# rferguson22/Gaussian-Process

Hardware: AMD Instinct MI355X
Metric: PSO objective evals/sec (swarm x iters) at N=4096 d=3 (higher is better)
Workload: dtype f64; 1 GPU; PSO objective, BASELINE config C: synthetic N=4096 d=3, swarm 64/GPU x 1 GPU = 64; N=4096, d=3, swarm=64, swarm_per_gpu=64, global_batch=64, seq_len=4096, parallelism=single GPU, hetero_noise=False, particles=interior l~U[0.05,0.6]^d (full work)

## Files before the change

gaussian-process_amd/csrc/gpf_common.hip:

```cpp
#pragma once

#include <hip/hip_runtime.h>
#include <stdint.h>

#include <utility>

namespace gpf {

typedef double d4 __attribute__((ext_vector_type(4)));
typedef double d2 __attribute__((ext_vector_type(2)));

constexpr int NTHR = 256;
constexpr int DNTH = 512;
constexpr int T = 128;
constexpr int DMAX = 32;
constexpr int KGRID_MAX = 4096;

__device__ __forceinline__ d4 mfma(double a, double b, d4 c) {
  return __builtin_amdgcn_mfma_f64_16x16x4f64(a, b, c, 0, 0, 0);
}

template <int TM> struct TileCfg;
template <> struct TileCfg<128> {
  static constexpr int KC = 16, NW = 8, WR = 1, WC = 8;
};

template <int TM> struct Geo {
  static constexpr int KC = TileCfg<TM>::KC;
  static constexpr int NW = TileCfg<TM>::NW;
  static constexpr int WR = TileCfg<TM>::WR;
  static constexpr int WC = TileCfg<TM>::WC;
  static constexpr int NTH = 64 * NW;
  static constexpr int MBR = TM / WR / 16;
  static constexpr int MBC = TM / WC / 16;
  static_assert(WR * WC == NW, "wave grid");
};

template <int TM> struct Quad {
  int lane, rb, cb;
  __device__ Quad() {
    const int tid = threadIdx.x;
    lane = tid & 63;
    const int w = __builtin_amdgcn_readfirstlane(tid >> 6);
    if constexpr (Geo<TM>::WR == 1) {
      rb = 0;
      cb = (w >= 4 ? 11 - w : w) * (TM / Geo<TM>::WC);
    } else {
      const int wr = w / Geo<TM>::WC, wc = w % Geo<TM>::WC;
      rb = wr * (TM / Geo<TM>::WR);
      cb = ((wr & 1) ? (Geo<TM>::WC - 1 - wc) : wc) * (TM / Geo<TM>::WC);
    }
  }
  __device__ __forceinline__ int row(int mi, int r) const { return rb + mi * 16 + (lane >> 4) + 4 * r; }
  __device__ __forceinline__ int col(int ni) const { return cb + ni * 16 + (lane & 15); }
};

template <typename P>
__device__ __forceinline__ P* launder(P* p) {
  using G = __attribute__((address_space(1))) P*;
  G g = (G)p;
  asm volatile("" : "+v"(g));
  return (P*)g;
}

template <int TM> struct Acc {
  static constexpr int MBR = Geo<TM>::MBR, MBC = Geo<TM>::MBC;
  d4 v[MBR][MBC];
  __device__ __forceinline__ void zero() {
#pragma unroll
    for (int i = 0; i < MBR; ++i)
#pragma unroll
      for (int j = 0; j < MBC; ++j) v[i][j] = d4{0.0, 0.0, 0.0, 0.0};
  }
  template <typename F>
  __device__ __forceinline__ void foreach(const Quad<TM>& q, F f) const {
#pragma unroll
    for (int mi = 0; mi < MBR; ++mi)
#pragma unroll
      for (int ni = 0; ni < MBC; ++ni)
#pragma unroll
        for (int r = 0; r < 4; ++r) f(q.row(mi, r), q.col(ni), v[mi][ni][r]);
  }
  __device__ __forceinline__ void load(const Quad<TM>& q, const double* base, size_t ld) {
    const double* p0 = launder(base + (size_t)(q.rb + (q.lane >> 4)) * ld + q.cb + (q.lane & 15));
#pragma unroll
    for (int mi = 0; mi < MBR; ++mi)
#pragma unroll
      for (int ni = 0; ni < MBC; ++ni)
#pragma unroll
        for (int r = 0; r < 4; ++r) v[mi][ni][r] = p0[(size_t)(mi * 16 + 4 * r) * ld + ni * 16];
  }
  __device__ __forceinline__ void store(const Quad<TM>& q, double* base, size_t ld) const {
    double* p0 = launder(base + (size_t)(q.rb + (q.lane >> 4)) * ld + q.cb + (q.lane & 15));
#pragma unroll
    for (int mi = 0; mi < MBR; ++mi)
#pragma unroll
      for (int ni = 0; ni < MBC; ++ni)
#pragma unroll
        for (int r = 0; r < 4; ++r) p0[(size_t)(mi * 16 + 4 * r) * ld + ni * 16] = v[mi][ni][r];
  }
  __device__ __forceinline__ void store_wt(const Quad<TM>& q, double* base, size_t ld) const {
    using G = __attribute__((address_space(1))) unsigned long long*;
    G p0 = (G)launder(base + (size_t)(q.rb + (q.lane >> 4)) * ld + q.cb + (q.lane & 15));
#pragma unroll
    for (int mi = 0; mi < MBR; ++mi)
#pragma unroll
      for (int ni = 0; ni < MBC; ++ni)
#pragma unroll
        for (int r = 0; r < 4; ++r)
          __hip_atomic_store(p0 + (size_t)(mi * 16 + 4 * r) * ld + ni * 16,
                             (unsigned long long)__double_as_longlong(v[mi][ni][r]), __ATOMIC_RELAXED,
                             __HIP_MEMORY_SCOPE_AGENT);
  }
  template <typename F>
  __device__ __forceinline__ void visit(const Quad<TM>& q, double* base, size_t ld, F f) const {
    double* p0 = launder(base + (size_t)(q.rb + (q.lane >> 4)) * ld + q.cb + (q.lane & 15));
#pragma unroll
    for (int mi = 0; mi < MBR; ++mi)
#pragma unroll
      for (int ni = 0; ni < MBC; ++ni)
#pragma unroll
        for (int r = 0; r < 4; ++r) f(p0[(size_t)(mi * 16 + 4 * r) * ld + ni * 16], v[mi][ni][r]);
  }
};

enum Tri : int {
  TRI_NONE = 0,
  TRI_B_KLEC,
  TRI_B_KGEC,
  TRI_A_KLER,
  TRI_C_LOWER,
  TRI_A_LAST,
};

template <int TRI>
__device__ __forceinline__ bool tri_live(int R0, int C0, int k) {
  if (TRI == TRI_B_KLEC) return k <= C0 + 15;
  if (TRI == TRI_B_KGEC) return k + 3 >= C0;
  if (TRI == TRI_A_KLER) return k <= R0 + 15;
  if (TRI == TRI_C_LOWER) return C0 <= R0 + 15;
  return true;
}

constexpr int DL_KC = 16;
constexpr int DL_BUF = 2 * 128 * DL_KC;
constexpr int DL_STAGE = 2 * DL_BUF;

__device__ __forceinline__ d4 mfma_neg_a(double a, double b, d4 c) {
  return __builtin_amdgcn_mfma_f64_16x16x4f64(a, b, c, 0, 0, 1);
}

__device__ __forceinline__ void dl_load(const double* g, double* l) {
  const uint32_t m = (uint32_t)(uintptr_t)(__attribute__((address_space(3))) void*)l;
  asm volatile("s_nop 0\n\tglobal_load_lds_dwordx4 %0, off" ::"v"(g), "{m0}"(m) : "memory");
}
template <bool NT = false>
__device__ __forceinline__ void dl_load_s(const void* base, uint32_t off, double* l) {
  const uint32_t m = (uint32_t)(uintptr_t)(__attribute__((address_space(3))) void*)l;
  if constexpr (NT)
    asm volatile("s_nop 0\n\tglobal_load_lds_dwordx4 %0, %1 nt" ::"v"(off), "s"(base), "{m0}"(m) : "memory");
  else
    asm volatile("s_nop 0\n\tglobal_load_lds_dwordx4 %0, %1" ::"v"(off), "s"(base), "{m0}"(m) : "memory");
}
#ifndef GPF_SUM_SHFL
#define GPF_SUM_SHFL 0
#endif
#ifndef GPF_B_NT
#define GPF_B_NT 1
#endif

__device__ __forceinline__ int dl_sw(int r) { return (r >> 1) & 7; }

template <typename P>
__device__ __forceinline__ P* uniform_ptr(P* p) {
  const unsigned long long v = (unsigned long long)(uintptr_t)p;
  const unsigned lo = __builtin_amdgcn_readfirstlane((unsigned)v), hi = __builtin_amdgcn_readfirstlane((unsigned)(v >> 32));
  return (P*)(uintptr_t)(((unsigned long long)hi << 32) | lo);
}

__device__ __forceinline__ void dl_row_offsets(int lane, uint32_t (&o)[4]) {
  const int lr = lane & 15, lk = lane >> 4;
#pragma unroll
  for (int s = 0; s < 4; ++s) o[s] = 8u * (uint32_t)(lr * DL_KC + 2 * ((2 * s + (lk >> 1)) ^ dl_sw(lr)) + (lk & 1));
}

template <bool NN, bool NEG, int NS = 2, bool BNT = true, bool TN = false>
struct DenseRun {
  static_assert(NS >= 2 && NS <= 4, "DenseRun stages");
  static_assert(!TN || NN, "TN: both operands are [k][c] panels");
  static constexpr int MBR = Geo<128>::MBR;
  static_assert(Geo<128>::MBC == 1 && Geo<128>::WR == 1, "128-tile wave layout: all rows x one column slab");
  uint32_t la[4], lb[4];
  uint32_t ga[2], gb[2];
  int blk0;

  __device__ __forceinline__ DenseRun(const Quad<128>& qd, int lda, int ldb, int wave) {
    const int lane = qd.lane, lr = lane & 15, lk = lane >> 4;
    if constexpr (TN) {
#pragma unroll
      for (int mi = 0; mi < 4; ++mi) la[mi] = 8u * (uint32_t)(lk * 128 + 2 * (8 * (mi ^ lk) + (lr >> 1)) + (lr & 1));
    } else {
      dl_row_offsets(lane, la);
    }
    if (!NN) {
#pragma unroll
      for (int s = 0; s < 4; ++s) lb[s] = la[s] + 8u * (uint32_t)(128 * DL_KC + qd.cb * DL_KC);
    } else {
      const int col = qd.cb + lr;
      lb[0] = 8u * (uint32_t)(128 * DL_KC + lk * 128 + 2 * ((col >> 1) ^ (8 * (lk & 3))) + (col & 1));
      lb[1] = lb[2] = lb[3] = lb[0];
    }
    blk0 = 2 * wave;
#pragma unroll
    for (int u = 0; u < 2; ++u) {
      const int blk = blk0 + u, row = 8 * blk + (lane >> 3), kp = (lane & 7) ^ dl_sw(row);
      ga[u] = TN ? 8u * (uint32_t)(blk * ldb + 2 * (lane ^ (8 * (blk & 3)))) : 8u * (uint32_t)(row * lda + 2 * kp);
      gb[u] = NN ? 8u * (uint32_t)(blk * ldb + 2 * (lane ^ (8 * (blk & 3)))) : 8u * (uint32_t)(row * ldb + 2 * kp);
    }
  }

  template <int BUF>
  __device__ __forceinline__ void issue(const double* Ap, const double* Bp, int ldb, int c, double* smem) const {
    const char* Ac = uniform_ptr(TN ? (const char*)(Ap + (size_t)c * DL_KC * ldb) : (const char*)(Ap + c * DL_KC));
    const char* Bc = uniform_ptr(NN ? (const char*)(Bp + (size_t)c * DL_KC * ldb) : (const char*)(Bp + c * DL_KC));
    double* sbuf = smem + BUF * DL_BUF;
#pragma unroll
    for (int u = 0; u < 2; ++u) {
      const int blk = blk0 + u;
      dl_load_s(Ac, ga[u], sbuf + (TN ? blk * 128 : blk * 8 * DL_KC));
      dl_load_s<BNT && GPF_B_NT != 0>(Bc, gb[u], sbuf + 128 * DL_KC + (NN ? blk * 128 : blk * 8 * DL_KC));
    }
  }

  template <int M0>
  __device__ __forceinline__ void reads(const char* sb, int s, double (&a)[MBR], double& b) const {
#pragma unroll
    for (int mi = M0; mi < MBR; ++mi) {
      if constexpr (TN) a[mi] = *(const double*)(sb + la[mi & 3] + (mi >> 2) * 64 * 8 + s * 512 * 8);
      else a[mi] = *(const double*)(sb + la[s] + mi * 16 * DL_KC * 8);
    }
    b = NN ? *(const double*)(sb + lb[0] + s * 512 * 8) : *(const double*)(sb + lb[s]);
  }

  template <int BUF, int M0>
  __device__ __forceinline__ void mma(Acc<128>& acc, const double* smem) const {
    if constexpr (M0 >= MBR) return;
    const char* sb = (const char*)smem + BUF * DL_BUF * 8;
    double a[MBR], b;
    reads<M0>(sb, 0, a, b);
#pragma unroll
    for (int s = 0; s < 4; ++s) {
#pragma unroll
      for (int mi = M0; mi < MBR; ++mi) acc.v[mi][0] = NEG ? mfma_neg_a(a[mi], b, acc.v[mi][0]) : mfma(a[mi], b, acc.v[mi][0]);
      if (s < 3) reads<M0>(sb, s + 1, a, b);
    }
  }

  template <int BUF, int M0>
  __device__ __forceinline__ void chunk(Acc<128>& acc, const double* Ap, const double* Bp, int ldb, int t, int nch,
                                        double* smem) const {
    if constexpr (NS == 2) {
      asm volatile("s_waitcnt vmcnt(0)" ::: "memory");
    } else {
      if (t + NS - 2 < nch) {
        if constexpr (NS == 3) asm volatile("s_waitcnt vmcnt(4)" ::: "memory");
        else asm volatile("s_waitcnt vmcnt(8)" ::: "memory");
      } else {
        asm volatile("s_waitcnt vmcnt(0)" ::: "memory");
      }
    }
    __syncthreads();
    if (t + NS - 1 < nch) issue<(BUF + NS - 1) % NS>(Ap, Bp, ldb, t + NS - 1, smem);
    mma<BUF, M0>(acc, smem);
  }
  template <int M0>
  __device__ __forceinline__ void chunk_rt(int b, Acc<128>& acc, const double* Ap, const double* Bp, int ldb, int t,
                                           int nch, double* smem) const {
    switch (b) {
      case 0: chunk<0, M0>(acc, Ap, Bp, ldb, t, nch, smem); break;
      case 1: chunk<1 % NS, M0>(acc, Ap, Bp, ldb, t, nch, smem); break;
      case 2: chunk<2 % NS, M0>(acc, Ap, Bp, ldb, t, nch, smem); break;
      default: chunk<3 % NS, M0>(acc, Ap, Bp, ldb, t, nch, smem); break;
    }
  }

  template <int M0>
  __device__ __forceinline__ void run(Acc<128>& acc, const double* Ap, const double* Bp, int ldb, int t0, int t1,
                                      int nch, double* smem) const {
    int t = t0;
    if constexpr (NS == 2) {
      if (t < t1 && (t & 1)) chunk<1, M0>(acc, Ap, Bp, ldb, t++, nch, smem);
#pragma unroll 1
      for (; t + 1 < t1; t += 2) {
        chunk<0, M0>(acc, Ap, Bp, ldb, t, nch, smem);
        chunk<1, M0>(acc, Ap, Bp, ldb, t + 1, nch, smem);
      }
      if (t < t1) chunk<0, M0>(acc, Ap, Bp, ldb, t, nch, smem);
    } else {
#pragma unroll 1
      for (; t < t1 && t % NS != 0; ++t) chunk_rt<M0>(t % NS, acc, Ap, Bp, ldb, t, nch, smem);
#pragma unroll 1
      for (; t + NS - 1 < t1; t += NS) {
        chunk<0, M0>(acc, Ap, Bp, ldb, t, nch, smem);
        chunk<1, M0>(acc, Ap, Bp, ldb, t + 1, nch, smem);
        chunk<2 % NS, M0>(acc, Ap, Bp, ldb, t + 2, nch, smem);
        if constexpr (NS == 4) chunk<3, M0>(acc, Ap, Bp, ldb, t + 3, nch, smem);
      }
#pragma unroll 1
      for (; t < t1; ++t) chunk_rt<M0>(t % NS, acc, Ap, Bp, ldb, t, nch, smem);
    }
  }
};

template <bool NN, bool NEG = false, int TRI = TRI_NONE, int NS = 2, bool BNT = true, bool TN = false>
__device__ __forceinline__ void gemm_stream_dl(Acc<128>& acc, const double* __restrict__ Ap, int lda, const double* __restrict__ Bp,
                               int ldb, int K, double* smem, const Quad<128>& qd) {
  const int nch = K / DL_KC;
  if (nch <= 0) return;
  const int wave = __builtin_amdgcn_readfirstlane(threadIdx.x >> 6);
  const double* Ar = uniform_ptr(Ap);
  const double* Br = uniform_ptr(Bp);
  const DenseRun<NN, NEG, NS, BNT, TN> dr(qd, lda, ldb, wave);
  dr.template issue<0>(Ar, Br, ldb, 0, smem);
  if constexpr (NS >= 3) {
    if (nch > 1) dr.template issue<1>(Ar, Br, ldb, 1, smem);
    if constexpr (NS >= 4)
      if (nch > 2) dr.template issue<2>(Ar, Br, ldb, 2, smem);
  }
  __builtin_amdgcn_s_waitcnt(0x0F70);
#define GPF_RUN(m0, a, b) dr.template run<m0>(acc, Ar, Br, ldb, (a), (b), nch, smem)
  const int slab = qd.cb / 16;
  if constexpr (TRI == TRI_NONE) {
    GPF_RUN(0, 0, nch);
// ... 78 lines not shown
#pragma unroll
  for (int mi = M0; mi < 8; ++mi)
#pragma unroll
    for (int r = 0; r < 4; ++r) {
      double* q = p1 + (size_t)(mi * 16 + 4 * r) * ldc;
      if (WT)
        __hip_atomic_store(reinterpret_cast<unsigned long long*>(q),
                           (unsigned long long)__double_as_longlong(acc.v[mi][0][r]), __ATOMIC_RELAXED,
                           __HIP_MEMORY_SCOPE_AGENT);
      else
        *q = acc.v[mi][0][r];
    }
}

template <bool WT>
__device__ __forceinline__ void syrk_tile(double* __restrict__ C, size_t ldc, const double* __restrict__ A, int lda,
                                          int K, double* smem, const Quad<128>& qd) {
  switch (qd.cb / 16) {
    case 0: syrk_rows<WT, 0>(C, ldc, A, lda, K, smem, qd); break;
    case 1: syrk_rows<WT, 1>(C, ldc, A, lda, K, smem, qd); break;
    case 2: syrk_rows<WT, 2>(C, ldc, A, lda, K, smem, qd); break;
    case 3: syrk_rows<WT, 3>(C, ldc, A, lda, K, smem, qd); break;
    case 4: syrk_rows<WT, 4>(C, ldc, A, lda, K, smem, qd); break;
    case 5: syrk_rows<WT, 5>(C, ldc, A, lda, K, smem, qd); break;
    case 6: syrk_rows<WT, 6>(C, ldc, A, lda, K, smem, qd); break;
    default: syrk_rows<WT, 7>(C, ldc, A, lda, K, smem, qd); break;
  }
}

constexpr int TRI_LD = 17;
constexpr int TRI_LDS = 36 * 16 * TRI_LD;
__host__ __device__ constexpr int tri_chunk(int m) { return 16 * TRI_LD * (8 * m - m * (m - 1) / 2); }

__device__ __forceinline__ int tri_row_chunk(int ri, int& rr) {
  int m = 0, base = 0;
#pragma unroll
  for (int mm = 0; mm < 7; ++mm)
    if (ri >= base + 16 * (8 - m)) {
      base += 16 * (8 - m);
      ++m;
    }
  rr = ri - base;
  return m;
}
struct NoHook {
  __device__ void operator()() const {}
};
#ifndef GPF_TRI_STAGE_SCALAR
#define GPF_TRI_STAGE_SCALAR 1
#endif
__host__ __device__ __forceinline__ void tri_block(int b, int& m, int& rb) {
  m = 0;
  int base = 0;
#pragma unroll
  for (int mm = 0; mm < 7; ++mm)
    if (b >= base + (8 - m)) {
      base += 8 - m;
      ++m;
    }
  rb = m + (b - base);
}
template <typename Hook = NoHook>
__device__ __forceinline__ void tri_to_lds(const double* __restrict__ U, size_t ld, double* s, Hook hook = Hook()) {
#if GPF_TRI_STAGE_SCALAR
  {
    const int tid = threadIdx.x;
    const int grp = __builtin_amdgcn_readfirstlane(tid >> 7);
    const int r = (tid >> 3) & 15, kp = tid & 7;
    const double* ul = U + (size_t)r * ld + 2 * kp;
    d2 v[9];
#pragma unroll
    for (int u = 0; u < 9; ++u) {
      int m, rb;
      tri_block(grp + 4 * u, m, rb);
      v[u] = *reinterpret_cast<const d2*>(ul + (size_t)(16 * rb) * ld + 16 * m);
    }
    if constexpr (!__is_same(Hook, NoHook)) {
      asm volatile("s_waitcnt vmcnt(0)" ::: "memory");
      hook();
    }
    double* sl = s + r * TRI_LD + 2 * kp;
#pragma unroll
    for (int u = 0; u < 9; ++u) {
      int m, rb;
      tri_block(grp + 4 * u, m, rb);
      const int off = tri_chunk(m) + 16 * (rb - m) * TRI_LD;
      sl[off] = v[u].x;
      sl[off + 1] = v[u].y;
    }
    __syncthreads();
    return;
  }
#endif
  int tid = threadIdx.x;
  d2 v[9];
#pragma unroll
  for (int u = 0; u < 9; ++u) {
    const int i = tid + DNTH * u, ri = i >> 3, kp = i & 7;
    int rr;
    const int m = tri_row_chunk(ri, rr);
    v[u] = *reinterpret_cast<const d2*>(U + (size_t)(16 * m + rr) * ld + 16 * m + 2 * kp);
  }
  if constexpr (!__is_same(Hook, NoHook)) {
    asm volatile("s_waitcnt vmcnt(0)" ::: "memory");
    hook();
  }
  asm volatile("" : "+v"(tid));
#pragma unroll
  for (int u = 0; u < 9; ++u) {
    const int i = tid + DNTH * u, ri = i >> 3, kp = i & 7;
    int rr;
    const int m = tri_row_chunk(ri, rr);
    const int dst = tri_chunk(m) + rr * TRI_LD + 2 * kp;
    s[dst] = v[u].x;
    s[dst + 1] = v[u].y;
  }
  __syncthreads();
}

template <int P, bool NEG>
__device__ __forceinline__ void trmm_acc(d4 (&out)[2], const Acc<128>& X, const double* sU) {
  constexpr int NQ = 4 * (2 * P + 2);
  const int lane = threadIdx.x & 63;
  const uint32_t b0 = 8u * (uint32_t)((lane & 15) * TRI_LD + (lane >> 4));
  uint32_t b1 = b0 + 32768u;
  asm volatile("" : "+v"(b1));
  const char* u = (const char*)sU;
  out[0] = d4{0.0, 0.0, 0.0, 0.0};
  out[1] = d4{0.0, 0.0, 0.0, 0.0};
  double a[2][2];
  auto reads = [&](int q, double (&r)[2]) {
    const int mi = q >> 2, e = q & 3;
#pragma unroll
    for (int j = 0; j < 2; ++j)
      if (2 * P + j >= mi) {
        const int off = 8 * (tri_chunk(mi) + (2 * P + j - mi) * 16 * TRI_LD + 4 * e);
        r[j] = off < 32768 ? *(const double*)(u + b0 + off) : *(const double*)(u + b1 + (off - 32768));
      }
  };
  reads(0, a[0]);
#pragma unroll
  for (int q = 0; q < NQ; ++q) {
    if (q + 1 < NQ) reads(q + 1, a[(q + 1) & 1]);
    __builtin_amdgcn_sched_barrier(0);
    const int mi = q >> 2, e = q & 3;
#pragma unroll
    for (int j = 0; j < 2; ++j)
      if (2 * P + j >= mi)
        out[j] = NEG ? mfma_neg_a(a[q & 1][j], X.v[mi][0][e], out[j]) : mfma(a[q & 1][j], X.v[mi][0][e], out[j]);
    __builtin_amdgcn_sched_barrier(0);
  }
}

template <bool WT = false>
__device__ __forceinline__ void gst(double* p, double v) {
  if (WT)
    __hip_atomic_store(reinterpret_cast<unsigned long long*>(p), (unsigned long long)__double_as_longlong(v),
                       __ATOMIC_RELAXED, __HIP_MEMORY_SCOPE_AGENT);
  else
    *p = v;
}

struct ClockSpan {
  unsigned long long* s;
  __device__ __forceinline__ explicit ClockSpan(unsigned long long* lds2) : s(lds2) {}
  __device__ __forceinline__ void start(const unsigned long long* clk) const {
    if (clk && threadIdx.x == 0) {
      unsigned long long t0, r0;
      asm volatile("s_memtime %0\n\ts_waitcnt lgkmcnt(0)" : "=s"(t0)::"memory");
      asm volatile("s_memrealtime %0\n\ts_waitcnt lgkmcnt(0)" : "=s"(r0)::"memory");
      s[0] = t0;
      s[1] = r0;
    }
  }
  __device__ __forceinline__ void stop(unsigned long long* clk) const {
    if (clk && threadIdx.x == 0) {
      unsigned long long t1, r1;
      asm volatile("s_memtime %0\n\ts_waitcnt lgkmcnt(0)" : "=s"(t1)::"memory");
      asm volatile("s_memrealtime %0\n\ts_waitcnt lgkmcnt(0)" : "=s"(r1)::"memory");
      __hip_atomic_fetch_add(clk, t1 - s[0], __ATOMIC_RELAXED, __HIP_MEMORY_SCOPE_AGENT);
      __hip_atomic_fetch_add(clk + 1, r1 - s[1], __ATOMIC_RELAXED, __HIP_MEMORY_SCOPE_AGENT);
    }
  }
};

template <int ROWS>
__device__ __forceinline__ double add_swapped(double v) {
  const unsigned long long u = __builtin_bit_cast(unsigned long long, v);
  const unsigned lo = (unsigned)u, hi = (unsigned)(u >> 32);
  unsigned a0, a1, b0, b1;
  if constexpr (ROWS == 16) {
    const auto a = __builtin_amdgcn_permlane16_swap(lo, lo, false, false);
    const auto b = __builtin_amdgcn_permlane16_swap(hi, hi, false, false);
    a0 = a[0], a1 = a[1], b0 = b[0], b1 = b[1];
  } else {
    const auto a = __builtin_amdgcn_permlane32_swap(lo, lo, false, false);
    const auto b = __builtin_amdgcn_permlane32_swap(hi, hi, false, false);
    a0 = a[0], a1 = a[1], b0 = b[0], b1 = b[1];
  }
  const double x = __builtin_bit_cast(double, ((unsigned long long)b0 << 32) | a0);
  const double y = __builtin_bit_cast(double, ((unsigned long long)b1 << 32) | a1);
  return x + y;
}

__device__ __forceinline__ double sum_lane_groups(double v) {
#if GPF_SUM_SHFL
  v = v + __shfl_xor(v, 16);
  v = v + __shfl_xor(v, 32);
  return v;
#else
  return add_swapped<32>(add_swapped<16>(v));
#endif
}

}
```

gaussian-process_amd/csrc/gpf_factor.hip:

```cpp

#pragma once
#include "gpf_common.hip"
#include "gpf_diag.hip"

namespace gpf {

__global__ __launch_bounds__(DNTH) void k_diag(int J, int nt, int N, int Npad, double* __restrict__ Lb,
                                                  double* __restrict__ Ub, double* __restrict__ yb,
                                                  double* __restrict__ s2p, double* __restrict__ szp,
                                                  int* __restrict__ info, int* __restrict__ dflag) {
  if (threadIdx.x == 0) dflag[blockIdx.x] = J;
  __shared__ __attribute__((aligned(16))) double lds[DB_LDS];
  const int p = blockIdx.x;
  const size_t ld = (size_t)Npad;
  const size_t off = (size_t)p * ld * ld + (size_t)J * T * ld + (size_t)J * T;
  const size_t poff = ((size_t)p * nt + J) * Npad + (size_t)J * T;
  factor128(Lb + off, Ub + off, ld, yb + (size_t)p * Npad + J * T, s2p + poff, szp + poff, info + p, lds);
  (void)N;
}

__host__ __device__ __forceinline__ void step_tile(int b, int P, int ntl, int grp, int& p, int& w) {
  if ((P & 7) != 0 || grp <= 0) {
    p = b % P;
    w = b / P;
// ... 686 lines not shown

__host__ __device__ __forceinline__ int lall_head(int P, int nt, int nstd) { return nstd - P * (nt - 1); }
__host__ __device__ __forceinline__ bool lall_is_piece(int b, int J, int P, int nt, int nstd, int bits, int tag) {
  if (!(bits & 4)) return b >= nstd;
  const int h = lall_head(P, nt, nstd);
  return b >= h && b < h + P * lall_total(J, nt, pb_of(tag));
}
__host__ __device__ __forceinline__ int lall_piece_index(int b, int P, int nt, int nstd, int bits) {
  return (bits & 4) ? b - lall_head(P, nt, nstd) : b - nstd;
}
__host__ __device__ __forceinline__ int lall_tile_block(int b, int J, int P, int nt, int nstd, int tag) {
  return b < lall_head(P, nt, nstd) ? b : b - P * lall_total(J, nt, pb_of(tag));
}
__device__ __forceinline__ void add_node(Acc<T>& acc, const double* slot) {
  const auto rs = __builtin_amdgcn_make_buffer_rsrc((void*)uniform_ptr(slot), 0, T * T * 8, 0x00020000);
  const int wb = __builtin_amdgcn_readfirstlane(threadIdx.x >> 6) * NODE_WAVE, lane = threadIdx.x & 63;
#pragma unroll
  for (int mi = 0; mi < Acc<T>::MBR; ++mi)
#pragma unroll
    for (int h = 0; h < 2; ++h) {
      const d2 v = __builtin_bit_cast(d2, __builtin_amdgcn_raw_buffer_load_b128(rs, lane * 16, wb + (mi * 2 + h) * 1024, 0));
      acc.v[mi][0][2 * h] = acc.v[mi][0][2 * h] + v.x;
      acc.v[mi][0][2 * h + 1] = acc.v[mi][0][2 * h + 1] + v.y;
    }
}
__device__ __forceinline__ void lall_seed(Acc<T>& acc, const double* lb, int J, int it, int p, int tag, int nt) {
  const int P = P_of(tag), smax = smax_of(tag), pb = pb_of(tag);
  const int np = lall_np(J - 1, it, nt, pb);
  const double* s0 = lb + lall_slot(J - 1, it, 0, p, P, nt, smax, pb);
  load_node(acc, s0);
  for (int s = 1; s < np; ++s) add_node(acc, s0 + (size_t)s * T * T);
}

__device__ __forceinline__ void lall_piece(int J, int it, int s, int p, int nt, int Npad, const double* __restrict__ Lb,
                                           const double* __restrict__ Ub, int N, const double* __restrict__ x,
                                           const double* __restrict__ ls, int d, double* __restrict__ lb, int tag,
                                           double* lds) {
  const size_t ld = (size_t)Npad;
  const int pb = pb_of(tag);
  const int nLc = nt - 2 - J, depth = lall_depth(J, it, nt);
  const int b0 = s * pb, nb = min(pb, depth - b0);
  const double* Lp = Lb + (size_t)p * ld * ld;
  const Quad<T> qd;
  Acc<T> acc;
  if (it < nLc) {
    const int I = J + 2 + it;
    if (s == 0) cov_tile_acc(acc, qd, x, ls + (size_t)p * d, d, N, J + 1, I, lds);
    else acc.zero();
    gemm_stream_dl<false, true>(acc, Lp + (size_t)(J + 1) * T * ld + (size_t)b0 * T, Npad,
                                Lp + (size_t)I * T * ld + (size_t)b0 * T, Npad, nb * T, lds, qd);
  } else if (it < nLc + J) {
    const int K = it - nLc;
    const double* Up = Ub + (size_t)p * ld * ld;
    const double* A = Lp + (size_t)(J + 1) * T * ld + (size_t)(K + b0) * T;
    const double* B = Up + (size_t)(K + b0) * T * ld + (size_t)K * T;
    acc.zero();
    if (s == 0) gemm_stream_dl<true, false, TRI_B_KGEC>(acc, A, Npad, B, Npad, nb * T, lds, qd);
    else gemm_stream_dl<true, false>(acc, A, Npad, B, Npad, nb * T, lds, qd);
  } else {
    const double* Ar = Lp + (size_t)(J + 2) * T * ld + (size_t)b0 * T;
    if (s == 0) acc.load(qd, Lp + (size_t)(J + 2) * T * ld + (size_t)(J + 2) * T, ld);
    else acc.zero();
    gemm_stream_dl<false, true>(acc, Ar, Npad, Ar, Npad, nb * T, lds, qd);
  }
  store_node(acc, lb + lall_slot(J, it, s, p, P_of(tag), nt, smax_of(tag), pb), qd);
}

__device__ __forceinline__ void lall_syrk_item(int J, int p, int nt, int Npad, double* __restrict__ Lb,
                                               int* __restrict__ yflag, const double* __restrict__ lb, int tag,
                                               double* lds) {
  const size_t ld = (size_t)Npad;
  const int I = J + 1;
  double* Lp = Lb + (size_t)p * ld * ld;
  const Quad<T> qd;
  Acc<T> acc;
  lall_seed(acc, lb, J, nt - 2, p, tag, nt);
  const double* Ar = Lp + (size_t)I * T * ld + (size_t)(J - 1) * T;
  gemm_stream_dl<false, true>(acc, Ar, Npad, Ar, Npad, T, lds, qd);
  acc.store_wt(qd, Lp + (size_t)I * T * ld + (size_t)I * T, ld);
  asm volatile("s_waitcnt vmcnt(0)" ::: "memory");
  __syncthreads();
  if (threadIdx.x == 0) __hip_atomic_store(yflag + p, J, __ATOMIC_RELAXED, __HIP_MEMORY_SCOPE_AGENT);
}

__device__ __forceinline__ void tile_st(double* p, double v) { *p = v; }

template <int SPLIT, int ED>
__device__ __forceinline__ void step_item(int role, int J, int w, int p, int nt, int Npad, double* __restrict__ Lb,
                                          double* __restrict__ Ub, double* __restrict__ yb,
                                          double* __restrict__ s2p, double* __restrict__ szp,
                                          int* __restrict__ info, int N, const double* __restrict__ x,
                                          const double* __restrict__ ls, int d, int S, int S2, int sidx,
                                          double* __restrict__ part, unsigned* __restrict__ cnt, int* sflag,
                                          const int* __restrict__ dflag, const int* __restrict__ yflag, int defer,
                                          int spins, int la, const double* __restrict__ lab, int pair,
                                          const double* __restrict__ pb, int ptag, double* lds) {
  const int tid = threadIdx.x;
  const int nL = nt - 1 - J;
  constexpr bool PAIRS = SPLIT == SPLIT_NONE && !ED;
  const bool follow = PAIRS && pair == 2;
  constexpr bool LALL = SPLIT == SPLIT_NONE && ED;
  const bool lseed = LALL && (pair & 2) && J >= 2;
  const size_t ld = (size_t)Npad;
  if (SPLIT != SPLIT_NONE && role == ROLE_IDLE) return;
  double* Lp = Lb + (size_t)p * ld * ld;
  double* Up = Ub + (size_t)p * ld * ld;
  double* yp = yb + (size_t)p * Npad;
  if constexpr (SPLIT == SPLIT_ALL) {
    static_assert(ED, "the all-tile split runs with the early diagonal factor (host: early_diag)");
    const int np = split_all_pieces(J, w, nt, S);
if (w < nL)
      flat_piece<true>(J, w, p, nt, Npad, Lp, Up, yp, s2p, szp, info + p, N, x, ls + (size_t)p * d, d, np, sidx, S2, part,
                       cnt, sflag, dflag, spins, lds);
    else
      flat_piece<false>(J, w, p, nt, Npad, Lp, Up, yp, s2p, szp, info + p, N, x, ls + (size_t)p * d, d, np, sidx, S2, part,
                        cnt, sflag, dflag, spins, lds);
    return;
  }
  const Quad<T> qd;
  const int g = qd.lane >> 4, cl = qd.lane & 15;
  const double* Ujj = Up + (size_t)J * T * ld + (size_t)J * T;
  double* zj = lds + STEP_ZJ;

  if (w < nL) {
    const int I = J + 1 + w;
    double* Aij = Lp + (size_t)I * T * ld + (size_t)J * T;
    double* Aii = Lp + (size_t)I * T * ld + (size_t)I * T;
    const double* lp = ls + (size_t)p * d;
    Acc<T> acc;
    if (SPLIT == SPLIT_NONE && ED && (la & 2) && I == J + 1) {
      const int k0 = la_chunks(J - 1) * DL_KC;
      if (la & 4) {
        for (int i = 0; i < 96; ++i) __builtin_amdgcn_s_sleep(127);
        __syncthreads();
      }
      acc.load(qd, lab + la_slot(p, J - 1), T);
      gemm_stream_dl<false, true>(acc, Lp + (size_t)J * T * ld + k0, Npad, Lp + (size_t)I * T * ld + k0, Npad, J * T - k0,
                                  lds, qd);
    } else if (lseed) {
      lall_seed(acc, pb, J, w, p, ptag, nt);
      gemm_stream_dl<false, true>(acc, Lp + (size_t)J * T * ld + (size_t)(J - 1) * T, Npad,
                                  Lp + (size_t)I * T * ld + (size_t)(J - 1) * T, Npad, T, lds, qd);
    } else if (follow) {
      load_node(acc, pb + pair_slot(p, w, nt));
      gemm_stream_dl<false, true>(acc, Lp + (size_t)J * T * ld + (size_t)(J - 1) * T, Npad,
                                  Lp + (size_t)I * T * ld + (size_t)(J - 1) * T, Npad, T, lds, qd);
    } else {
      cov_tile_acc(acc, qd, x, lp, d, N, J, I, lds);
      if (J > 0)
        gemm_stream_dl<false, true>(acc, Lp + (size_t)J * T * ld, Npad, Lp + (size_t)I * T * ld, Npad, J * T, lds, qd);
    }
    GPF_PHASE(0);
    if (ED && wait_diag(dflag + p, J, info + p, spins, sflag)) return;
    if (tid < T) zj[tid] = yp[J * T + tid];
    tri_to_lds(Ujj, ld, lds);
    GPF_PHASE(3);
    double* lrow = launder(Aij + (size_t)(qd.cb + cl) * ld + g);
    double yr = 0.0;
#pragma unroll
    for (int P = 0; P < 4; ++P) {
      d4 o[2];
      switch (P) {
        case 0: trmm_acc<0, false>(o, acc, lds); break;
        case 1: trmm_acc<1, false>(o, acc, lds); break;
        case 2: trmm_acc<2, false>(o, acc, lds); break;
        default: trmm_acc<3, false>(o, acc, lds); break;
      }
#pragma unroll
      for (int j = 0; j < 2; ++j)
#pragma unroll
        for (int e = 0; e < 4; ++e) {
          tile_st(&lrow[16 * (2 * P + j) + 4 * e], o[j][e]);
          yr = fma(o[j][e], zj[16 * (2 * P + j) + 4 * e + g], yr);
        }
    }
    yr = sum_lane_groups(yr);
    if (g == 0) yp[I * T + qd.cb + cl] = yp[I * T + qd.cb + cl] - yr;
    GPF_PHASE(1);
    __syncthreads();
    const bool defer_on = SPLIT != SPLIT_ALL && defer;
    if (follow && I == J + 1) {
      syrk_tile<false>(Aii, ld, Aij - T, Npad, 2 * T, lds, qd);
    } else if (!defer_on || I == J + 1) {
      if (defer_on && J > 0 && wait_diag(yflag + p, J, info + p, spins, sflag)) return;
      syrk_tile<false>(Aii, ld, Aij, Npad, T, lds, qd);
    }
    GPF_PHASE(2);
    if (!ED && I == J + 1) {
      __syncthreads();
      const size_t poff = ((size_t)p * nt + I) * Npad + (size_t)I * T;
      __builtin_amdgcn_s_setprio(3);
      factor128(Aii, Up + (size_t)I * T * ld + (size_t)I * T, ld, yp + I * T, s2p + poff, szp + poff, info + p, lds);
    }
  } else {
    const int K = w - nL;
    double* Ujk = Up + (size_t)J * T * ld + (size_t)K * T;
    Acc<T> acc;
    if (lseed && K < J - 1) {
      lall_seed(acc, pb, J, w, p, ptag, nt);
      gemm_stream_dl<true, false>(acc, Lp + (size_t)J * T * ld + (size_t)(J - 1) * T, Npad,
                                  Up + (size_t)(J - 1) * T * ld + (size_t)K * T, Npad, T, lds, qd);
    } else if (follow && K < J - 1) {
      load_node(acc, pb + pair_slot(p, w, nt));
      gemm_stream_dl<true, false>(acc, Lp + (size_t)J * T * ld + (size_t)(J - 1) * T, Npad,
                                  Up + (size_t)(J - 1) * T * ld + (size_t)K * T, Npad, T, lds, qd);
    } else {
      acc.zero();
      gemm_stream_dl<true, false, TRI_B_KGEC>(acc, Lp + (size_t)J * T * ld + (size_t)K * T, Npad,
                                              Up + (size_t)K * T * ld + (size_t)K * T, Npad, (J - K) * T, lds, qd);
    }
    GPF_PHASE(0);
    if (ED && wait_diag(dflag + p, J, info + p, spins, sflag)) return;
    if (tid < T) zj[tid] = yp[J * T + tid];
#ifdef GPF_WG_TRACE
    tri_to_lds(Ujj, ld, lds, [&] { GPF_PHASE(2); });
#else
    tri_to_lds(Ujj, ld, lds);
#endif
    GPF_PHASE(3);
    double* ucol = launder(Ujk + (size_t)g * ld + qd.cb + cl);
    double a2[2] = {0.0, 0.0}, az[2] = {0.0, 0.0};
#pragma unroll
    for (int P = 0; P < 4; ++P) {
      d4 o[2];
      switch (P) {
        case 0: trmm_acc<0, true>(o, acc, lds); break;
        case 1: trmm_acc<1, true>(o, acc, lds); break;
        case 2: trmm_acc<2, true>(o, acc, lds); break;
        default: trmm_acc<3, true>(o, acc, lds); break;
      }
      const int h = P >> 1;
#pragma unroll
      for (int j = 0; j < 2; ++j)
#pragma unroll
        for (int e = 0; e < 4; ++e) {
          const int row = 16 * (2 * P + j) + 4 * e;
          const double v = o[j][e];
          tile_st(&ucol[(size_t)row * ld], v);
          a2[h] = fma(v, v, a2[h]);
          az[h] = fma(v, zj[row + g], az[h]);
        }
    }
#pragma unroll
    for (int h = 0; h < 2; ++h) {
      a2[h] = sum_lane_groups(a2[h]);
      az[h] = sum_lane_groups(az[h]);
    }
    GPF_PHASE(1);
    if (g == 0) {
      const size_t poff = ((size_t)p * nt + J) * Npad + (size_t)K * T + qd.cb + cl;
      s2p[poff] = a2[0] + a2[1];
      szp[poff] = az[0] + az[1];
    }
  }
}

template <int SPLIT, int ED>
__global__ __launch_bounds__(STEP_NTH, SPLIT == SPLIT_ALL ? 2 : STEP_WAVES_PER_SIMD) void k_step(int J, int nt, int Npad, double* __restrict__ Lb,
                                                  double* __restrict__ Ub, double* __restrict__ yb,
                                                  double* __restrict__ s2p, double* __restrict__ szp,
                                                  int* __restrict__ info, int P, int grp, int N,
                                                  const double* __restrict__ x, const double* __restrict__ ls,
                                                  int d, int S, int S2, double* __restrict__ part,
                                                  unsigned* __restrict__ cnt, int* __restrict__ dflag, int ed,
                                                  int* __restrict__ yflag, int defer, int sy, int spins, int la,
                                                  double* __restrict__ lab, int pair, double* __restrict__ pb,
                                                  int* __restrict__ pstart, int ptag,
                                                  unsigned long long* __restrict__ clk) {
  const int tid = threadIdx.x;
  __shared__ unsigned long long sclk[2];
  const ClockSpan span(sclk);
  span.start(clk);
#ifdef GPF_WG_TRACE
  if (tid == 0 && J < WG_TRACE_J && blockIdx.x < WG_TRACE_N) {
    unsigned hw, xcc;
    asm volatile("s_getreg_b32 %0, hwreg(HW_REG_HW_ID)" : "=s"(hw));
    asm volatile("s_getreg_b32 %0, hwreg(HW_REG_XCC_ID)" : "=s"(xcc));
    g_wg_trace[J][blockIdx.x][0] = realtime();
    g_wg_trace[J][blockIdx.x][2] = ((unsigned long long)xcc << 32) | hw;
  }
#endif
  __shared__ __attribute__((aligned(16))) double lds[SPLIT == SPLIT_ALL ? STEP_LDS_FLAT : STEP_LDS];
  __shared__ int sflag;
  int p, w, sidx = 0;
  constexpr bool PAIRS = SPLIT == SPLIT_NONE && !ED;
  int uh = 0, lit = -1;
  constexpr bool LALL = SPLIT == SPLIT_NONE && ED;
  const int nstd = (ED && ed ? P : 0) + (SPLIT != SPLIT_ALL && sy ? P : 0) + P * (nt - 1);
  int role;
  if (PAIRS && pair == 1) {
    role = pair_decode((int)blockIdx.x, J, P, nt, p, w, &uh);
  } else if (LALL && (pair & 1) && lall_is_piece((int)blockIdx.x, J, P, nt, nstd, pair, ptag)) {
    lall_decode(lall_piece_index((int)blockIdx.x, P, nt, nstd, pair), J, P, nt, pb_of(ptag), p, lit, sidx);
    w = -1;
    role = ROLE_LPIECE;
  } else {
    role = step_decode<SPLIT>(LALL && (pair & 5) == 5 ? lall_tile_block((int)blockIdx.x, J, P, nt, nstd, ptag) : (int)blockIdx.x, J,
                              P, nt, grp, S, ED && ed, SPLIT != SPLIT_ALL && sy,
                              SPLIT == SPLIT_NONE && ED && (la & 1) && !sy, p, w, sidx,
                              SPLIT == SPLIT_NONE && ED && (la & 32) != 0);
  }
#ifdef GPF_CHECK
  {
    bool ok = p >= 0 && p < P && J >= 0 && J < nt && Npad == nt * T && S >= 1 && S2 >= 1 && S2 <= SPLIT_MAXS;
    if (role == ROLE_SYRK) ok = ok && w == -1 && J >= 1 && J <= nt - 2 && yflag != nullptr;
    else if (role == ROLE_LA) ok = ok && w == -1 && J >= 1 && J + 2 < nt && lab != nullptr;
    else if (role == ROLE_DIAG) ok = ok && w == -1 && ED && dflag != nullptr;
    else if (role == ROLE_PLA) ok = ok && PAIRS && pair == 1 && pb != nullptr && w >= 1 && w < nt - 1 && J >= 1 &&
                                     (w >= nt - 1 - J || J + 1 + w < nt);
    else if (role == ROLE_SYRKP) ok = ok && PAIRS && pair == 1 && w == 1 && J >= 1 && J + 2 <= nt - 1;
    else if (role == ROLE_LPIECE) ok = ok && LALL && pb != nullptr && lit >= 0 && lit < lall_items(J, nt) && sidx >= 0 &&
                                       sidx < lall_np(J, lit, nt, pb_of(ptag)) && P_of(ptag) == P &&
                                       lall_off(J, lit, nt, pb_of(ptag)) + sidx < smax_of(ptag);
    else if (role != ROLE_IDLE) ok = ok && w >= 0 && w < nt - 1 && sidx >= 0 && (pair != 2 || pb != nullptr) &&
                                     sidx < (SPLIT == SPLIT_ALL ? split_all_pieces(J, w, nt, S) : S) && sidx < S2 &&
                                     (role != ROLE_PIECE || (part != nullptr && cnt != nullptr && S > 1)) &&
                                     (w >= nt - 1 - J || J + 1 + w < nt) && (w < nt - 1 - J || w - (nt - 1 - J) < J);
    if (!ok) {
      if (tid == 0)
        printf("k_step check: J=%d block %d role %d p=%d w=%d sidx=%d (P=%d nt=%d S=%d)\n", J, (int)blockIdx.x, role,
               p, w, sidx, P, nt, S);
      return;
    }
  }
#endif
  if (PAIRS && pair == 1 && pstart) pair_start_sync(J, role == ROLE_SYRK ? 0 : w, uh, p, nt, pstart, ptag);
  if (LALL && role == ROLE_LPIECE) {
    lall_piece(J, lit, sidx, p, nt, Npad, Lb, Ub, N, x, ls, d, pb, ptag, lds);
  } else if (LALL && role == ROLE_SYRK && (pair & 2) && J >= 2) {
    lall_syrk_item(J, p, nt, Npad, Lb, yflag, pb, ptag, lds);
  } else if (PAIRS && role == ROLE_PLA) {
    pla_item(J, w, p, nt, Npad, Lb, Ub, N, x, ls, d, pb, lds);
  } else if (PAIRS && role == ROLE_SYRKP) {
    syrkp_item(J, p, Npad, Lb, lds);
  } else if (SPLIT != SPLIT_ALL && role == ROLE_SYRK) {
    syrk_item(J, p, Npad, Lb, yflag, lds);
    if (SPLIT == SPLIT_NONE && ED && (la & 1)) {
      __syncthreads();
      la_item(J, p, Npad, Lb, N, x, ls, d, lab, lds);
    }
  } else if (SPLIT == SPLIT_NONE && ED && role == ROLE_LA) {
    la_item(J, p, Npad, Lb, N, x, ls, d, lab, lds);
  } else if (ED && role == ROLE_DIAG) {
    const size_t ld = (size_t)Npad;
    const size_t off = (size_t)p * ld * ld + (size_t)J * T * ld + (size_t)J * T;
    const size_t poff = ((size_t)p * nt + J) * Npad + (size_t)J * T;
    __builtin_amdgcn_s_setprio(3);
    factor128<true>(Lb + off, Ub + off, ld, yb + (size_t)p * Npad + J * T, s2p + poff, szp + poff, info + p, lds,
                    dflag + p, J);
  } else {
    step_item<SPLIT, ED>(role, J, w, p, nt, Npad, Lb, Ub, yb, s2p, szp, info, N, x, ls, d, S, S2, sidx, part, cnt, &sflag,
                         dflag, yflag, defer, spins, la, lab, pair, pb, ptag, lds);
  }
  span.stop(clk);
#ifdef GPF_WG_TRACE
  __syncthreads();
  if (tid == 0 && J < WG_TRACE_J && blockIdx.x < WG_TRACE_N) g_wg_trace[J][blockIdx.x][1] = realtime();
#endif
}


__global__ __launch_bounds__(DNTH) void k_debug_factor128(double* __restrict__ L, double* __restrict__ U,
                                                          double* __restrict__ y, double* __restrict__ s2,
                                                          double* __restrict__ sz, int* __restrict__ bad,
                                                          unsigned long long* __restrict__ cyc) {
  __shared__ __attribute__((aligned(16))) double lds[DB_LDS];
  const int b = blockIdx.x;
  unsigned long long t0 = 0, t1 = 0;
  __syncthreads();
  asm volatile("s_memtime %0\n\ts_waitcnt lgkmcnt(0)" : "=s"(t0)::"memory");
  factor128(L + (size_t)b * T * T, U + (size_t)b * T * T, T, y + (size_t)b * T, s2 + (size_t)b * T, sz + (size_t)b * T,
            bad + b, lds);
  asm volatile("s_waitcnt vmcnt(0)" ::: "memory");
  __syncthreads();
  asm volatile("s_memtime %0\n\ts_waitcnt lgkmcnt(0)" : "=s"(t1)::"memory");
  if (cyc && threadIdx.x == 0) cyc[b] = t1 - t0;
}

__global__ __launch_bounds__(NTHR) void k_fill_hash(double* __restrict__ p, long long n) {
  for (long long i = blockIdx.x * (long long)NTHR + threadIdx.x; i < n; i += (long long)gridDim.x * NTHR) {
    unsigned long long h = (unsigned long long)i * 0x9e3779b97f4a7c15ull;
    h ^= h >> 31;
    h *= 0xbf58476d1ce4e5b9ull;
    h ^= h >> 29;
    p[i] = (double)(h >> 11) * 0x1.0p-52 - 1.0;
  }
}

template <int NS>
__global__ __launch_bounds__(STEP_NTH, NS >= 3 ? 2 : STEP_WAVES_PER_SIMD) void k_gemm_bench(int mode, int D, int Npad, int P,
                                                                                   const double* __restrict__ Lb,
                                                                                   double* __restrict__ C,
                                                                                   unsigned long long* clk) {
  __shared__ __attribute__((aligned(16))) double smem[NS * DL_BUF];
  __shared__ unsigned long long cs[2];
// ... 21 lines not shown
```

Measured before the change: 1403 evals/s.

## Stream triangular diagonal block into LDS by slabs and overlap TRMM with loads

Replaces the full tri_to_lds staging followed by TRMM with a slab-wise streamed TRMM. Blocks of the diagonal upper-triangular tile are async-loaded straight to LDS in reverse slab order, and multiplication starts as soon as the first slabs arrive, using graded vmcnt waits. Row stores are interleaved with the remaining multiplies, and the z_J vector load rides on the same async path. This hides the global-to-LDS staging latency behind MFMA work, at the cost of complex offset bookkeeping, extra barriers and correctness risk in the slab indexing.

```diff
diff --git a/gaussian-process_amd/csrc/gpf_common.hip b/gaussian-process_amd/csrc/gpf_common.hip
--- a/gaussian-process_amd/csrc/gpf_common.hip
+++ b/gaussian-process_amd/csrc/gpf_common.hip
@@ -169,7 +169,7 @@
 #define GPF_B_NT 1
 #endif
 
-__device__ __forceinline__ int dl_sw(int r) { return (r >> 1) & 7; }
+__host__ __device__ constexpr int dl_sw(int r) { return (r >> 1) & 7; }
 
 template <typename P>
 __device__ __forceinline__ P* uniform_ptr(P* p) {
@@ -178,7 +178,7 @@
   return (P*)(uintptr_t)(((unsigned long long)hi << 32) | lo);
 }
 
-__device__ __forceinline__ void dl_row_offsets(int lane, uint32_t (&o)[4]) {
+__host__ __device__ __forceinline__ void dl_row_offsets(int lane, uint32_t (&o)[4]) {
   const int lr = lane & 15, lk = lane >> 4;
 #pragma unroll
   for (int s = 0; s < 4; ++s) o[s] = 8u * (uint32_t)(lr * DL_KC + 2 * ((2 * s + (lk >> 1)) ^ dl_sw(lr)) + (lk & 1));
@@ -563,6 +563,148 @@
   }
 }
 
+#ifndef GPF_FINISH_STAGED
+#define GPF_FINISH_STAGED 0
+#endif
+constexpr int SLAB_BLK = 16 * DL_KC;
+constexpr int SLAB_IMG = 36 * SLAB_BLK;
+static_assert(SLAB_IMG <= TRI_LDS, "the slab image fits the staged form's area (z_J follows it)");
+__host__ __device__ constexpr int slab_first(int s) { return 72 - (s + 1) * (s + 2); }
+__host__ __device__ constexpr int slab_m0(int s, int wave) { return ((wave >> 1) - (slab_first(s) >> 1)) & 3; }
+__host__ __device__ constexpr int slab_count(int s, int wave) {
+  return (slab_m0(s, wave) <= s ? 1 : 0) + (slab_m0(s, wave) + 4 <= s ? 1 : 0);
+}
+__host__ __device__ constexpr int slab_later(int s, int wave) {
+  int n = 0;
+  for (int q = 0; q < s; ++q) n += slab_count(q, wave);
+  return n;
+}
+__host__ __device__ constexpr uint32_t slab_src(int wave, int lane, int ld) {
+  const int row = 8 * (wave & 1) + (lane >> 3);
+  return 8u * (uint32_t)(row * ld + 2 * ((lane & 7) ^ dl_sw(row)));
+}
+__host__ __device__ constexpr int slab_base(int s) {
+  return s == 3 ? 32 * SLAB_BLK : SLAB_BLK * (36 - (s + 1) * (s + 2) / 2 - (s < 3 ? 4 : 0));
+}
+__host__ __device__ constexpr int slab_dst(int s, int m, int wave) { return slab_base(s) + m * SLAB_BLK + (wave & 1) * 8 * DL_KC; }
+__host__ __device__ constexpr uint32_t slab_read(int s, int mi) { return 8u * (uint32_t)(slab_base(s) + mi * SLAB_BLK); }
+
+__device__ __forceinline__ void vm_wait(int n) {
+  switch (n) {
+    case 0: asm volatile("s_waitcnt vmcnt(0)" ::: "memory"); break;
+    case 1: asm volatile("s_waitcnt vmcnt(1)" ::: "memory"); break;
+    case 2: asm volatile("s_waitcnt vmcnt(2)" ::: "memory"); break;
+    case 3: asm volatile("s_waitcnt vmcnt(3)" ::: "memory"); break;
+    case 4: asm volatile("s_waitcnt vmcnt(4)" ::: "memory"); break;
+    case 5: asm volatile("s_waitcnt vmcnt(5)" ::: "memory"); break;
+    case 6: asm volatile("s_waitcnt vmcnt(6)" ::: "memory"); break;
+    default: asm volatile("s_waitcnt vmcnt(7)" ::: "memory"); break;
+  }
+}
+
+template <bool NEG, int B, int NB>
+__device__ __forceinline__ void slab_mult(Acc<128>& X, const char* rb, const uint32_t (&la)[4]) {
+  static_assert(NB == 1 || (NB == 2 && B >= 1), "one block or a pair");
+  constexpr int NQ = 4 * (B + 1);
+  constexpr bool HIGH = slab_read(B, B) >= 65536u || slab_read(B - NB + 1, 0) >= 65536u;
+  uint32_t lh[4] = {0, 0, 0, 0};
+  if constexpr (HIGH) {
+#pragma unroll
+    for (int e = 0; e < 4; ++e) {
+      lh[e] = la[e] + 65536u;
+      asm volatile("" : "+v"(lh[e]));
+    }
+  }
+  d4 t[NB];
+#pragma unroll
+  for (int j = 0; j < NB; ++j) t[j] = d4{0.0, 0.0, 0.0, 0.0};
+  if constexpr (NB == 1) {
+    double g[2][4];
+    auto reads4 = [&](int mi, double (&r)[4]) {
+#pragma unroll
+      for (int e = 0; e < 4; ++e) {
+        const uint32_t off = slab_read(B, mi);
+        r[e] = off < 65536u ? *(const double*)(rb + la[e] + off) : *(const double*)(rb + lh[e] + (off - 65536u));
+      }
+    };
+    reads4(0, g[0]);
+#pragma unroll
+    for (int mi = 0; mi <= B; ++mi) {
+      if (mi < B) reads4(mi + 1, g[(mi + 1) & 1]);
+      __builtin_amdgcn_sched_barrier(0);
+#pragma unroll
+      for (int e = 0; e < 4; ++e) t[0] = NEG ? mfma_neg_a(g[mi & 1][e], X.v[mi][0][e], t[0]) : mfma(g[mi & 1][e], X.v[mi][0][e], t[0]);
+      __builtin_amdgcn_sched_barrier(0);
+    }
+    X.v[B][0] = t[0];
+    return;
+  }
+  double a[2][NB];
+  auto reads = [&](int q, double (&r)[NB]) {
+    const int mi = q >> 2, e = q & 3;
+#pragma unroll
+    for (int j = 0; j < NB; ++j)
+      if (B - j >= mi) {
+        const uint32_t off = slab_read(B - j, mi);
+        r[j] = off < 65536u ? *(const double*)(rb + la[e] + off) : *(const double*)(rb + lh[e] + (off - 65536u));
+      }
+  };
+  reads(0, a[0]);
+#pragma unroll
+  for (int q = 0; q < NQ; ++q) {
+    if (q + 1 < NQ) reads(q + 1, a[(q + 1) & 1]);
+    __builtin_amdgcn_sched_barrier(0);
+    const int mi = q >> 2, e = q & 3;
+#pragma unroll
+    for (int j = 0; j < NB; ++j)
+      if (B - j >= mi) t[j] = NEG ? mfma_neg_a(a[q & 1][j], X.v[mi][0][e], t[j]) : mfma(a[q & 1][j], X.v[mi][0][e], t[j]);
+    __builtin_amdgcn_sched_barrier(0);
+  }
+#pragma unroll
+  for (int j = 0; j < NB; ++j) X.v[B - j][0] = t[j];
+}
+
+template <bool NEG, typename Store, typename Hook = NoHook>
+__device__ __forceinline__ void trmm_stream(Acc<128>& X, const double* __restrict__ U, int ld, const double* zsrc,
+                                            double* zdst, double* img, Store store, Hook hook = Hook()) {
+  const int lane = threadIdx.x & 63;
+  const int wave = __builtin_amdgcn_readfirstlane(threadIdx.x >> 6);
+  const uint32_t go = slab_src(wave, lane, ld);
+  uint32_t la[4];
+  dl_row_offsets(lane, la);
+  if (wave == 7) dl_load(zsrc + 2 * lane, zdst);
+#pragma unroll
+  for (int s = 7; s >= 0; --s) {
+    const int m0 = slab_m0(s, wave);
+#pragma unroll
+    for (int j = 0; j < 2; ++j) {
+      const int m = m0 + 4 * j;
+      if (m <= s) dl_load_s(uniform_ptr((const char*)(U + (size_t)(16 * s) * ld + 16 * m)), go, img + slab_dst(s, m, wave));
+    }
+  }
+  const char* rb = (const char*)img;
+  vm_wait(slab_later(7, wave));
+  __syncthreads();
+  hook();
+  slab_mult<NEG, 7, 1>(X, rb, la);
+  vm_wait(slab_later(5, wave));
+  __syncthreads();
+  slab_mult<NEG, 6, 2>(X, rb, la);
+  vm_wait(0);
+  __syncthreads();
+  store(7);
+  store(6);
+  store(5);
+  slab_mult<NEG, 4, 2>(X, rb, la);
+  store(4);
+  store(3);
+  slab_mult<NEG, 2, 2>(X, rb, la);
+  store(2);
+  store(1);
+  slab_mult<NEG, 0, 1>(X, rb, la);
+  store(0);
+}
+
 template <bool WT = false>
 __device__ __forceinline__ void gst(double* p, double v) {
   if (WT)
diff --git a/gaussian-process_amd/csrc/gpf_factor.hip b/gaussian-process_amd/csrc/gpf_factor.hip
--- a/gaussian-process_amd/csrc/gpf_factor.hip
+++ b/gaussian-process_amd/csrc/gpf_factor.hip
@@ -862,11 +862,26 @@
     }
     GPF_PHASE(0);
     if (ED && wait_diag(dflag + p, J, info + p, spins, sflag)) return;
+    double* lrow = launder(Aij + (size_t)(qd.cb + cl) * ld + g);
+    double yr = 0.0;
+#if !GPF_FINISH_STAGED
+    auto lst = [&](int ib) {
+#pragma unroll
+      for (int e = 0; e < 4; ++e) tile_st(&lrow[16 * ib + 4 * e], acc.v[ib][0][e]);
+    };
+#ifdef GPF_WG_TRACE
+    trmm_stream<false>(acc, Ujj, Npad, yp + J * T, zj, lds, lst, [&] { GPF_PHASE(3); });
+#else
+    trmm_stream<false>(acc, Ujj, Npad, yp + J * T, zj, lds, lst);
+#endif
+#pragma unroll
+    for (int ib = 0; ib < 8; ++ib)
+#pragma unroll
+      for (int e = 0; e < 4; ++e) yr = fma(acc.v[ib][0][e], zj[16 * ib + 4 * e + g], yr);
+#else
     if (tid < T) zj[tid] = yp[J * T + tid];
     tri_to_lds(Ujj, ld, lds);
     GPF_PHASE(3);
-    double* lrow = launder(Aij + (size_t)(qd.cb + cl) * ld + g);
-    double yr = 0.0;
 #pragma unroll
     for (int P = 0; P < 4; ++P) {
       d4 o[2];
@@ -884,6 +899,7 @@
           yr = fma(o[j][e], zj[16 * (2 * P + j) + 4 * e + g], yr);
         }
     }
+#endif
     yr = sum_lane_groups(yr);
     if (g == 0) yp[I * T + qd.cb + cl] = yp[I * T + qd.cb + cl] - yr;
     GPF_PHASE(1);
@@ -921,6 +937,31 @@
     }
     GPF_PHASE(0);
     if (ED && wait_diag(dflag + p, J, info + p, spins, sflag)) return;
+    double* ucol = launder(Ujk + (size_t)g * ld + qd.cb + cl);
+    double a2[2] = {0.0, 0.0}, az[2] = {0.0, 0.0};
+#if !GPF_FINISH_STAGED
+    auto ust = [&](int ib) {
+#pragma unroll
+      for (int e = 0; e < 4; ++e) tile_st(&ucol[(size_t)(16 * ib + 4 * e) * ld], acc.v[ib][0][e]);
+    };
+#ifdef GPF_WG_TRACE
+    trmm_stream<true>(acc, Ujj, Npad, yp + J * T, zj, lds, ust, [&] {
+      GPF_PHASE(2);
+      GPF_PHASE(3);
+    });
+#else
+    trmm_stream<true>(acc, Ujj, Npad, yp + J * T, zj, lds, ust);
+#endif
+#pragma unroll
+    for (int ib = 0; ib < 8; ++ib)
+#pragma unroll
+      for (int e = 0; e < 4; ++e) {
+        const int row = 16 * ib + 4 * e;
+        const double v = acc.v[ib][0][e];
+        a2[ib >> 2] = fma(v, v, a2[ib >> 2]);
+        az[ib >> 2] = fma(v, zj[row + g], az[ib >> 2]);
+      }
+#else
     if (tid < T) zj[tid] = yp[J * T + tid];
 #ifdef GPF_WG_TRACE
     tri_to_lds(Ujj, ld, lds, [&] { GPF_PHASE(2); });
@@ -928,8 +969,6 @@
     tri_to_lds(Ujj, ld, lds);
 #endif
     GPF_PHASE(3);
-    double* ucol = launder(Ujk + (size_t)g * ld + qd.cb + cl);
-    double a2[2] = {0.0, 0.0}, az[2] = {0.0, 0.0};
 #pragma unroll
     for (int P = 0; P < 4; ++P) {
       d4 o[2];
@@ -951,6 +990,7 @@
           az[h] = fma(v, zj[row + g], az[h]);
         }
     }
+#endif
 #pragma unroll
     for (int h = 0; h < 2; ++h) {
       a2[h] = sum_lane_groups(a2[h]);
```

Result: no change. 1407 evals/s, median of 5 (+0.3%).
